# ChampiB/CBO_with_OOP

Hardware: AMD Instinct MI355X
Metric: candidate-intervention acquisitions/sec (16k grid, d=3) (higher is better)
Workload: dtype f64

## Files before the change

### cbo_with_oop_amd/GaussianProcessFactory.py

```python
from __future__ import annotations

import ctypes
import os
import warnings
from enum import IntEnum

import numpy as np

from . import _lib


class GaussianProcessType(IntEnum):
    GRAPH_GP = 0
    CAUSAL_GP = 1
    NON_CAUSAL_GP = 2


_LOGEXP_LIM = 36.0
_LOGEXP_LOG_LIM = float(np.log(np.finfo(np.float64).max))


def logexp_f(x):
    x = np.asarray(x, dtype=np.float64)
    return np.where(x > _LOGEXP_LIM, x, np.log1p(np.exp(np.clip(x, -_LOGEXP_LOG_LIM, _LOGEXP_LIM))))
# ... 93 lines not shown

    def _fit(self):
        tries = ctypes.c_int(0)
        jitter = ctypes.c_double(0.0)
        _lib.check(self._lib.cbo_gp_fit(self._handle, ctypes.byref(tries), ctypes.byref(jitter)))
        self._note_jitter(tries.value, jitter.value)

    def fit_level(self, level):
        status = ctypes.c_int(0)
        jitter = ctypes.c_double(0.0)
        _lib.check(self._lib.cbo_gp_fit_level(self._handle, int(level), ctypes.byref(status), ctypes.byref(jitter)))
        if status.value == 1:
            self._note_jitter(int(level), jitter.value)
        return status.value, jitter.value

    def adopted_factor(self, level):
        tries = ctypes.c_int(0)
        jitter = ctypes.c_double(0.0)
        _lib.check(self._lib.cbo_gp_jitter(self._handle, ctypes.byref(tries), ctypes.byref(jitter)))
        self._note_jitter(tries.value, jitter.value)

    def take_factor_slices(self, source, level, n_owners):
        _lib.check(self._lib.cbo_gp_take_factor_slices(self._handle, source._handle, int(level), int(n_owners)))
        self.adopted_factor(level)
        self.stale = False

    stale = False

    @property
    def small(self):
# ... 721 lines not shown
```

### cbo_with_oop_amd/_lib.py

```python
from __future__ import annotations

import atexit
import ctypes
import os
import threading
import weakref

import numpy as np

_HERE = os.path.dirname(os.path.abspath(__file__))
LIB_PATH = os.environ.get("CBO_HIP_LIB", os.path.join(_HERE, "libcbo_hip.so"))

c_double_p = ctypes.POINTER(ctypes.c_double)
c_int64_p = ctypes.POINTER(ctypes.c_int64)
c_int_p = ctypes.POINTER(ctypes.c_int)
c_void_pp = ctypes.POINTER(ctypes.c_void_p)

ABI_VERSION = 5
MAX_DIM = 8
MAX_APPEND = 64
MAX_HYPER_SAMPLES = 256
MAX_BATCH = 64
SMALL_BATCH_MAX_CANDS = 1024
CBO_OK = 0
# ... 222 lines not shown
    "cbo_acq_refine_sets_prior": (ctypes.c_int, [ctypes.c_int, c_void_pp, ctypes.POINTER(CboRefineSet), c_void_pp, ctypes.c_int,
                                                 c_double_p, ctypes.c_int, ctypes.c_double, ctypes.c_int, c_double_p, c_double_p,
                                                 c_double_p, c_int_p, c_int_p]),
    "cbo_do_prior_create": (ctypes.c_int, [ctypes.c_void_p, ctypes.c_int64, c_double_p, ctypes.c_int, c_int_p, c_void_pp]),
    "cbo_do_prior_destroy": (None, [ctypes.c_void_p]),
    "cbo_do_prior_eval": (ctypes.c_int, [ctypes.c_void_p, ctypes.c_int64, c_double_p, c_double_p, c_double_p]),
    "cbo_gp_hmc_sets": (ctypes.c_int, [ctypes.c_int, c_void_pp, ctypes.POINTER(CboHmcChain), c_int_p]),
    "cbo_gp_mle_sets": (ctypes.c_int, [ctypes.c_int, c_void_pp, ctypes.POINTER(CboMleRun), c_int_p]),
    "cbo_gp_mle_sets_rows": (ctypes.c_int, [ctypes.c_int, c_void_pp, ctypes.POINTER(CboMleRun), ctypes.c_int, c_int_p]),
    "cbo_gp_set_priors": (ctypes.c_int, [ctypes.c_void_p, ctypes.c_int, ctypes.POINTER(CboHyperPrior)]),
    "cbo_gp_get_priors": (ctypes.c_int, [ctypes.c_void_p, ctypes.c_int, ctypes.POINTER(CboHyperPrior)]),
    "cbo_gp_log_prior_batch": (ctypes.c_int, [ctypes.c_int, c_void_pp, ctypes.POINTER(c_double_p), c_double_p, c_double_p,
                                              c_int_p]),
    "cbo_gp_mes_gumbel_sets": (ctypes.c_int, [ctypes.c_int, c_void_pp, c_void_pp, c_double_p, c_double_p, c_double_p]),
    "cbo_gp_fit_level": (ctypes.c_int, [ctypes.c_void_p, ctypes.c_int, c_int_p, c_double_p]),
    "cbo_comm_gather_i64": (ctypes.c_int, [ctypes.c_void_p, ctypes.c_int64, c_int64_p]),
    "cbo_comm_share_factor": (ctypes.c_int, [ctypes.c_void_p, ctypes.c_void_p, ctypes.c_int, c_int_p, ctypes.c_int,
                                              c_int_p, ctypes.c_int]),
    "cbo_gp_take_factor_slices": (ctypes.c_int, [ctypes.c_void_p, ctypes.c_void_p, ctypes.c_int, ctypes.c_int]),
    "cbo_schedule_report": (ctypes.c_int, [ctypes.c_void_p, ctypes.c_char_p, ctypes.c_int64]),
    "cbo_trial_step": (ctypes.c_int, [ctypes.c_int, c_void_pp, c_void_pp, ctypes.c_int, ctypes.c_int64, c_double_p, c_double_p,
                                      c_double_p, c_double_p, c_double_p, ctypes.c_int, ctypes.c_double, c_double_p, c_double_p,
                                      c_int64_p, c_int_p]),
    "cbo_trial_step_kind": (ctypes.c_int, [ctypes.c_int, c_void_pp, c_void_pp, ctypes.c_int, ctypes.c_int64, c_double_p,
                                           c_double_p, c_double_p, c_double_p, ctypes.c_int, c_double_p, ctypes.c_int,
                                           ctypes.c_double, c_double_p, c_double_p, c_int64_p, c_int_p]),
    "cbo_acq_sweep_host": (ctypes.c_int, [ctypes.c_void_p, ctypes.c_int64, c_double_p, c_double_p, c_double_p,
                                          ctypes.c_double, ctypes.c_int, ctypes.c_double, ctypes.c_double,
                                          c_double_p, c_double_p, c_int64_p]),
    "cbo_argmax_sets": (ctypes.c_int, [c_double_p, ctypes.c_int, c_int_p]),
# ... 167 lines not shown
```

### cbo_with_oop_amd/csrc/cbo_api.hip

```cpp
#include <algorithm>
#include <atomic>
#include <cmath>
#include <cstdio>
#include <cstdlib>
#include <chrono>
#include <cstring>
#include <mutex>
#include <string>
#include <map>
#include <utility>
#include <vector>

#include "cbo_internal.h"
#include "hyper_prior.h"
#include "lml_outputs.h"
#include "schedule_tuner.h"

using namespace cbo;

static thread_local std::string g_err;
static std::atomic<uint64_t> g_fit_stamp{0};

static int fail(int code, const std::string &msg)
{
    g_err = msg;
    return code;
}
namespace cbo {
int set_error(int code, const std::string &msg) { return fail(code, msg); }
}

// ... 45 lines not shown
struct cbo_ctx {
    int device = 0;
    hipStream_t stream = nullptr;
    hipStream_t side_stream = nullptr;
    hipStream_t sweep_stream = nullptr;
    hipStream_t bulk_stream = nullptr;
    std::vector<hipEvent_t> chol_events;
    std::vector<hipEvent_t> pipe_events;
    hipEvent_t ev_join = nullptr, ev_join2 = nullptr, ev_fork = nullptr;
    hipEvent_t region_a = nullptr, region_b = nullptr;
    double pipe_tail_frac = -1.0;
    int pipe_group = 0;
    int pipe_lead = -1;
    CholOptions chol;
    int vec_solve_form = 2;
    int n_cu = 256;
    int n_cu_pipe = 256;
    ScheduleTable schedule;
    int64_t fused_fallbacks = 0;
    bool sweep_cache = true;
    bool small_sets = true;
    int sweep_mode = -1;
    int overlap_mode = -1;
    bool profiling = false;
    std::vector<EventPair> pending;
    EventPair pipe_cur{};
    std::vector<hipEvent_t> pool;
    cbo_timers timers{};
    GrowBuf<double> V;
    GrowBuf<double> W;
// ... 69 lines not shown
    double *y = nullptr, *ls_dev = nullptr;
    std::vector<double> ls;
    std::vector<double> h_pv;
    KernelHyper h{};
    double noise_var = 0.0;
    double *A = nullptr;
    double *invDt = nullptr;
    double *alpha = nullptr;
    double *z = nullptr;
    int *info = nullptr;
    bool fitted = false;
    uint64_t fit_stamp = 0;
    bool alpha_ready = false;
    int tries = 0;
    double jitter = 0.0;
    uint64_t parent_stamp = 0;
    double append_d = 0.0, append_zn = 0.0;
    double *lvec = nullptr;
    cbo_cands *probe = nullptr;
    int k_last = 1;
    int blk_side = 0;
    int64_t blk_rows = 0;
    double *blk_mem = nullptr;
    double *blk_B[2] = {nullptr, nullptr};
    double *blk_L22[2] = {nullptr, nullptr};
    double *blk_zb[2] = {nullptr, nullptr};
    double *blk_y[2] = {nullptr, nullptr};
    double *blk_Kbb[2] = {nullptr, nullptr};
    double *blk_part = nullptr;
    int *blk_status = nullptr;
// ... 207 lines not shown
    if (tf) c->pipe_tail_frac = std::atof(tf);
    const char *pg = std::getenv("CBO_HIP_PIPE_GROUP");
    if (pg) c->pipe_group = std::min(std::max(std::atoi(pg), 0), 4);
    const char *pl = std::getenv("CBO_HIP_PIPE_LEAD");
    if (pl) c->pipe_lead = std::atoi(pl);
    const char *pf = std::getenv("CBO_HIP_PANEL_FORM");
    if (pf && (std::atoi(pf) == 2 || std::atoi(pf) == 5)) c->chol.panel_form = std::atoi(pf);
    const char *sl = std::getenv("CBO_HIP_FUSED_SPIN_LIMIT");
    if (sl) c->chol.spin_limit = std::atoi(sl);
    const char *bg = std::getenv("CBO_HIP_BULK_GROUP");
    if (bg) c->chol.bulk_group = std::atoi(bg);
    const char *g4 = std::getenv("CBO_HIP_BULK_GROUP4_ROWS");
    if (g4) c->chol.group4_rows = std::atoi(g4);
    const char *vf = std::getenv("CBO_HIP_VEC_SOLVE_FORM");
    if (vf) c->vec_solve_form = std::atoi(vf);
    {
        static std::once_flag once;
        std::call_once(once, [] { std::atexit(shutdown_all_at_exit); });
        std::lock_guard<std::mutex> lock(g_live_mutex);
        g_live.push_back(c);
    }
    *out = c;
    return CBO_OK;
}

namespace cbo {
hipStream_t ctx_stream(cbo_ctx *c) { return c->stream; }
int ctx_device(cbo_ctx *c) { return c->device; }
}

// ... 242 lines not shown
{
    if (!g) return fail(CBO_ERR_INVALID, "gp is NULL");
    if (!g->fitted) return fail(CBO_ERR_NOT_FITTED, "gp is not fitted");
    if (tries_out) *tries_out = g->tries;
    if (jitter_out) *jitter_out = g->jitter;
    return CBO_OK;
}

static CholOptions chol_options(const cbo_ctx *c, bool separate)
{
    CholOptions o = c->chol;
    if (separate) o.panel_form = 2;
    return o;
}

static void enqueue_factor(cbo_gp *g, double jitter, bool separate)
{
    cbo_ctx *c = g->ctx;
    {
        PhaseScope ps(c, PH_KXX);
        launch_kxx(c->stream, g->X, g->h, g->noise_var + kGpyDiagJitter, jitter, g->A, g->lda, g->n_pad);
        launch_rhs(c->stream, g->y, g->X.pm, g->n, g->A, g->lda, g->n_pad, g->info, cholesky_info_ints(g->n_pad));
    }
    {
        PhaseScope ps(c, PH_CHOL);
        launch_cholesky(c->stream, c->side_stream, c->chol_events, g->A, g->lda, g->n_pad, g->invDt, g->info,
                        chol_options(c, separate), nullptr, true);
    }
}

static bool jitter_step(double base, int *tries, double *jitter)
{
    *jitter = *tries == 0 ? base : *jitter * 10.0;
    ++*tries;
    return *tries <= 5 && std::isfinite(*jitter);
}

static int next_jitter(cbo_gp *g, int *tries, double *jitter)
{
    double base = 0.0;
    if (*tries == 0) {
        long double sum = 0.0L;
        bool nonpos = false;
        for (int64_t i = 0; i < g->n; ++i) {
            const double dv = g->h.variance + (g->h_pv.empty() ? 0.0 : g->h_pv[i]) + (g->noise_var + kGpyDiagJitter);
            if (!(dv > 0.0)) nonpos = true;
            sum += (long double)dv;
        }
        if (nonpos) return fail(CBO_ERR_NONPOS_DIAG, "not pd: non-positive diagonal elements");
        base = (double)(sum / (long double)g->n) * 1e-6;
    }
// ... 9 lines not shown
        HIP_TRY(hipGetLastError());
        HIP_TRY(hipMemcpyAsync(c->h_info, info, sizeof(int), hipMemcpyDeviceToHost, c->stream));
        HIP_TRY(hipStreamSynchronize(c->stream));
        if (*c->h_info == kCholFusedTimeout) {
            if (separate)
                return fail(CBO_ERR_HIP, "a fused diagonal + panel launch gave up waiting, and so did the separate-launch repeat");
            separate = true;
            ++c->fused_fallbacks;
            continue;
        }
        *pd = *c->h_info == 0;
        return CBO_OK;
    }
}

static void mark_fitted(cbo_gp *g, int tries, double jitter)
{
    g->fitted = true;
    g->fit_stamp = ++g_fit_stamp;
    g->parent_stamp = 0;
    g->alpha_ready = false;
    g->tries = tries;
    g->jitter = jitter;
    if (g->ctx->profiling) g->ctx->timers.n_fit += 1;
}

static int adopt_factor(cbo_gp *g, int tries, double jitter)
{
    cbo_ctx *c = g->ctx;
    HIP_TRY(hipMemcpy2DAsync(g->z, sizeof(double), g->A + g->n_pad, sizeof(double) * g->lda, sizeof(double),
                             (size_t)g->n_pad, hipMemcpyDeviceToDevice, c->stream));
    HIP_TRY(hipGetLastError());
    mark_fitted(g, tries, jitter);
    return CBO_OK;
}

extern "C" int cbo_gp_fit(cbo_gp *g, int *tries_out, double *jitter_out)
{
    if (!g) return fail(CBO_ERR_INVALID, "gp is NULL");
    if (g->n <= 0 || g->n_pad <= 0) return fail(CBO_ERR_INVALID, "gp holds no data (a previous upload failed)");
    cbo_ctx *c = g->ctx;
    HIP_TRY(hipSetDevice(c->device));
    g->fitted = false;
    double jitter = 0.0;
    int tries = 0;
    for (;;) {
        bool pd = false;
        int rc = attempt_factor(c, g->info, [&](bool separate) { enqueue_factor(g, jitter, separate); }, &pd);
        if (rc != CBO_OK) return rc;
        if (pd) break;
        rc = next_jitter(g, &tries, &jitter);
        if (rc != CBO_OK) return rc;
    }
    const int rc = adopt_factor(g, tries, jitter);
    if (rc != CBO_OK) return rc;
    if (tries_out) *tries_out = tries;
    if (jitter_out) *jitter_out = jitter;
    return CBO_OK;
}

static int ladder_jitter(cbo_gp *g, int level, double *jitter)
{
    *jitter = 0.0;
    int tries = 0;
    while (tries < level) {
// ... 4 lines not shown
}

extern "C" int cbo_gp_fit_level(cbo_gp *g, int level, int *status, double *jitter_out)
{
    if (!g || !status) return fail(CBO_ERR_INVALID, "NULL argument");
    if (g->n <= 0 || g->n_pad <= 0) return fail(CBO_ERR_INVALID, "gp holds no data (a previous upload failed)");
    if (level < 0) return fail(CBO_ERR_INVALID, "level must be >= 0");
    cbo_ctx *c = g->ctx;
    HIP_TRY(hipSetDevice(c->device));
    g->fitted = false;
    double jitter = 0.0;
    int rc = ladder_jitter(g, level, &jitter);
    if (rc == CBO_ERR_NONPOS_DIAG) { *status = -1; return CBO_OK; }
    if (rc != CBO_OK) return rc;
    bool pd = false;
    rc = attempt_factor(c, g->info, [&](bool separate) { enqueue_factor(g, jitter, separate); }, &pd);
    if (rc != CBO_OK) return rc;
    *status = pd ? 1 : 0;
    if (jitter_out) *jitter_out = jitter;
    return pd ? adopt_factor(g, level, jitter) : CBO_OK;
}

namespace cbo {
int gp_factor_view(cbo_gp *g, double **A, int64_t *lda, int64_t *n_pad, double **invDt, cbo_ctx **ctx)
{
    if (!g) return fail(CBO_ERR_INVALID, "gp is NULL");
    if (g->n <= 0 || g->n_pad <= 0) return fail(CBO_ERR_INVALID, "gp holds no data");
    *A = g->A; *lda = g->lda; *n_pad = g->n_pad; *invDt = g->invDt; *ctx = g->ctx;
    return CBO_OK;
}
bool gp_is_fitted_at(const cbo_gp *g, int level) { return g && g->fitted && g->tries == level; }
int gp_adopt_received_factor(cbo_gp *g, int level)
{
    HIP_TRY(hipSetDevice(g->ctx->device));
    double jitter = 0.0;
// ... 1208 lines not shown
        mubuf = k->mu;
        k->fit_stamp = 0;
    }
    const bool speculate = qbuf == k->q;
    SweepPipe pipe = make_pipe(g, Vws, ldv, k->m_pad, qbuf, mubuf);
    pipe.group = choice.group;
    int pairs = choice.pairs;
    pipe.lead = 0;
    if (pipe.group >= 2 && pairs >= 1 && pairs * 256 < (int)g->n_pad)
        pipe.lead = forced ? (c->pipe_lead > 0 ? c->pipe_lead : 0) : (c->pipe_lead >= 0 ? c->pipe_lead : pairs % pipe.group);
    pipe.tail_begin = pairs * 256;
    if (pipe.tail_begin > (int)g->n_pad) pipe.tail_begin = (int)g->n_pad;
    double jitter = 0.0;
    int tries = 0;
    bool separate = false;
    for (;;) {
        HIP_TRY(hipEventRecord(c->ev_fork, c->stream));
        HIP_TRY(hipStreamWaitEvent(c->sweep_stream, c->ev_fork, 0));
        {
            PhaseScope ps(c, PH_KXX);
            launch_kxx(c->stream, g->X, g->h, g->noise_var + kGpyDiagJitter, jitter, g->A, g->lda, g->n_pad);
            launch_rhs(c->stream, g->y, g->X.pm, g->n, g->A, g->lda, g->n_pad, g->info, cholesky_info_ints(g->n_pad));
        }
        {
            PhaseScope ps(c, PH_KSTAR, c->sweep_stream);
            launch_kstar(c->sweep_stream, g->X, k->P, 0, k->m_pad, g->h, Vws, ldv, g->n_pad);
        }
        launch_zero_pair(c->sweep_stream, qbuf, mubuf, k->m_pad);
        {
            PhaseScope ps(c, PH_CHOL);
            launch_cholesky(c->stream, c->side_stream, c->chol_events, g->A, g->lda, g->n_pad, g->invDt, g->info,
                            chol_options(c, separate), &pipe, true);
        }
        HIP_TRY(hipEventRecord(c->ev_join, c->sweep_stream));
        HIP_TRY(hipStreamWaitEvent(c->stream, c->ev_join, 0));
        HIP_TRY(hipEventRecord(c->ev_join2, c->bulk_stream));
        HIP_TRY(hipStreamWaitEvent(c->stream, c->ev_join2, 0));
        HIP_TRY(hipGetLastError());
        if (speculate) {
            rc = enqueue_finish(g, k, y_best, task, ei_jitter, cost, acq_out, mean_out, var_out, qbuf, mubuf, true, false);
            if (rc != CBO_OK) return rc;
        } else {
            HIP_TRY(hipMemcpyAsync(c->h_info, g->info, sizeof(int), hipMemcpyDeviceToHost, c->stream));
        }
        HIP_TRY(hipStreamSynchronize(c->stream));
        if (*c->h_info == 0) break;
        if (*c->h_info == kCholFusedTimeout) {
            if (separate)
                return fail(CBO_ERR_HIP, "a fused diagonal + panel launch gave up waiting, and so did the separate-launch repeat");
            separate = true;
            ++c->fused_fallbacks;
            continue;
        }
        rc = next_jitter(g, &tries, &jitter);
        if (rc != CBO_OK) return rc;
    }
    mark_fitted(g, tries, jitter);
    if (tries_out) *tries_out = tries;
    if (jitter_out) *jitter_out = jitter;
    if (Vws != c->V) { k->v_stamp = g->fit_stamp; k->v_rows = g->n; }
    if (qbuf == k->q) k->fit_stamp = g->fit_stamp;
    if (speculate) {
        if (acq_out || mean_out || var_out) {
            rc = copy_posterior_out(c, k, acq_out, mean_out, var_out);
            if (rc != CBO_OK) return rc;
            HIP_TRY(hipStreamSynchronize(c->stream));
        }
        complete_finish(c, best_val, best_idx);
// ... 2849 lines not shown
```

### cbo_with_oop_amd/csrc/cbo_internal.h

```cpp
#pragma once

#include <hip/hip_runtime.h>
#include <cstddef>
#include <cstdint>
#include <string>
#include <vector>

#include "cbo_hip.h"

namespace cbo {

typedef double d4 __attribute__((ext_vector_type(4)));
typedef double d2 __attribute__((ext_vector_type(2)));

#if defined(__HIP_DEVICE_COMPILE__) || defined(__HIPCC__)
typedef __attribute__((address_space(3))) void *lds_ptr_t;
__device__ __forceinline__ void glds16(const double *gsrc, unsigned lds_dst)
{
    unsigned keep;
    asm volatile("s_mov_b32 %0, m0\n\ts_mov_b32 m0, %2\n\ts_nop 0\n\tglobal_load_lds_dwordx4 %1, off\n\ts_mov_b32 m0, %0"
                 : "=&s"(keep)
                 : "v"(gsrc), "s"(lds_dst)
                 : "memory");
}
// ... 112 lines not shown
    std::vector<hipEvent_t> *events;
    void (*mark)(void *user, hipStream_t st, int begin, double flops);
    void *user;
};
constexpr int kCholFlagSlots = 1024;
constexpr int kCholFusedTimeout = -2147483647 - 1;
constexpr int kFusedSpinLimit = 1 << 22;
struct CholOptions {
    int panel_form = 4;
    int spin_limit = kFusedSpinLimit;
    int bulk_group = 4;
    int group4_rows = 10240;
};
void launch_cholesky(hipStream_t s, hipStream_t side, std::vector<hipEvent_t> &events, double *A, int64_t lda,
                     int64_t n_pad, double *invDt, int *info_dev, const CholOptions &opt, const SweepPipe *pipe = nullptr,
                     bool info_zeroed = false);
inline int cholesky_info_ints(int64_t n_pad)
{
    const int np = (int)(n_pad / 128);
    return 2 * np <= kCholFlagSlots ? 1 + 2 * np : 1;
}
void sweep_pipe_pair(const SweepPipe &pipe, hipStream_t chain, const double *A, int64_t lda, const double *invDt,
                     int64_t n_pad, int p, int r0, int klen);
void sweep_pipe_tail(const SweepPipe &pipe, hipStream_t chain, const double *A, int64_t lda, const double *invDt,
                     int64_t n_pad, int pairs_done);
void launch_backsolve(hipStream_t s, const double *A, int64_t lda, int64_t n_pad, const double *invDt, double *alpha);
void launch_forward_vec(hipStream_t s, const double *A, int64_t lda, int64_t n_pad, const double *invDt, double *w,
                        double *out);
void launch_gather_column(hipStream_t s, const double *V, int64_t ldv, int64_t n_pad, double *dst);
bool launch_backsolve_chain(hipStream_t s, const double *A, int64_t lda, int64_t n_pad, const double *invDt,
                            const double *src, int64_t src_stride, double *work, double *out, int *info, int spin_limit,
// ... 362 lines not shown
```

### cbo_with_oop_amd/csrc/kernels_chol.hip

```cpp
#include <hip/hip_ext.h>
#include <climits>
#include <atomic>
#include <cstring>
#include <vector>

#include "cbo_mid_lml_device.h"

namespace cbo {

__global__ __launch_bounds__(256) void potrf_diag128_v2_kernel(double *A, int64_t lda, int r0, int rcol,
                                                               double *__restrict__ invDt, int *info,
                                                               double *__restrict__ zvec)
{
    extern __shared__ __align__(16) unsigned char smem_raw[];
    Diag2Shared &sh = *reinterpret_cast<Diag2Shared *>(smem_raw);
    if (__builtin_nontemporal_load(info) != 0) return;
    const int tid = threadIdx.x;
    const int lane = tid & 63;
    const int wave = __builtin_amdgcn_readfirstlane(tid >> 6);
    {
        const unsigned s0 = lds_byte_address(&sh.S[0][0]);
        const double *g = A + (int64_t)(r0 + wave * 32) * lda + r0 + lane * 2;
#pragma unroll 8
        for (int p = 0; p < 32; ++p) {
// ... 157 lines not shown
            for (int kk = 0; kk < 4; ++kk)
#pragma unroll
                for (int t = s + 1; t < 8; ++t) ub[kk][t] = coherent_load(Ub + (int64_t)(16 * s + 4 * kk) * lda + 16 * t);
        }
        const d4 nx = -x;
#pragma unroll
        for (int kk = 0; kk < 4; ++kk)
#pragma unroll
            for (int t = s + 1; t < 8; ++t) acc[t] = MFMA_F64(ub[kk][t], nx[kk], acc[t]);
    }
}

void launch_panel_fused(hipStream_t s, double *A, int64_t lda, int r0, int rcol, double *invDt, int *info, double *zvec,
                        int n_cols, int *flag, int spin_limit, hipEvent_t done = nullptr, bool split = false)
{
    if (!split) {
        hipExtLaunchKernelGGL(potrf_panel_fused_kernel, dim3(1u + (unsigned)(n_cols / kStrip)), dim3(256), sizeof(Diag2Shared),
                              s, nullptr, done, 0, A, lda, r0, rcol, invDt, info, zvec, r0 + 128, flag, spin_limit, 1);
        return;
    }
    hipLaunchKernelGGL(potrf_panel_fused_kernel, dim3(1u), dim3(256), sizeof(Diag2Shared), s, A, lda, r0, rcol, invDt, info,
                       zvec, r0 + 128, flag, spin_limit, 1);
    hipExtLaunchKernelGGL(potrf_panel_fused_kernel, dim3((unsigned)(n_cols / kStrip)), dim3(256), 0, s, nullptr, done, 0, A,
                          lda, r0, rcol, invDt, info, zvec, r0 + 128, flag, spin_limit, 0);
}

void launch_panel_trsm(hipStream_t s, double *A, int64_t lda, int r0, int col0, int n_cols, const double *invDt,
                       const int *skip_if, hipEvent_t done = nullptr)
{
    if (n_cols <= 0) { if (done) hipEventRecord(done, s); return; }
    hipExtLaunchKernelGGL(panel_trsm_kernel, dim3((unsigned)(n_cols / kStrip)), dim3(256), sizeof(PanelShared), s, nullptr,
// ... 375 lines not shown
    const double rows = (double)((int)n_pad - t0);
    if (pipe.mark) pipe.mark(pipe.user, chain, 1, rows * rows * (double)pipe.m_pad);
    launch_trsm_strips(chain, A + (int64_t)t0 * lda + t0, lda, invDt + (int64_t)(t0 / 16) * 256,
                       pipe.V + (int64_t)t0 * pipe.ldv, pipe.ldv, (int64_t)n_pad - t0, pipe.m_pad, pipe.zvec + t0, pipe.q,
                       pipe.mu, true, false);
    if (pipe.mark) pipe.mark(pipe.user, chain, 0, 0.0);
}

__global__ void zero_ints_kernel(int *p, int n)
{
    for (int i = threadIdx.x; i < n; i += blockDim.x) p[i] = 0;
}

void launch_cholesky(hipStream_t s, hipStream_t side, std::vector<hipEvent_t> &events, double *A, int64_t lda,
                     int64_t n_pad, double *invDt, int *info_dev, const CholOptions &opt, const SweepPipe *pipe,
                     bool info_zeroed)
{
    hipFuncSetAttribute(reinterpret_cast<const void *>(potrf_diag128_v2_kernel), hipFuncAttributeMaxDynamicSharedMemorySize,
                        (int)sizeof(Diag2Shared));
    hipFuncSetAttribute(reinterpret_cast<const void *>(panel_trsm_kernel), hipFuncAttributeMaxDynamicSharedMemorySize,
                        (int)sizeof(PanelShared));
    hipFuncSetAttribute(reinterpret_cast<const void *>(potrf_panel_fused_kernel), hipFuncAttributeMaxDynamicSharedMemorySize,
                        (int)sizeof(Diag2Shared));
    constexpr int syrk_gemm_rows = 6144;
    auto launch_diag = [&](int rr) {
        hipLaunchKernelGGL(potrf_diag128_v2_kernel, dim3(1), dim3(256), sizeof(Diag2Shared), s, A, lda, rr, (int)n_pad,
                           invDt, info_dev, pipe ? pipe->zvec : nullptr);
    };
    const int np = (int)(n_pad / 128);
    const bool fused = opt.panel_form != 2 && 2 * np <= kCholFlagSlots;
    const bool split = opt.panel_form == 5;
    if (!info_zeroed) hipLaunchKernelGGL(zero_ints_kernel, dim3(1), dim3(256), 0, s, info_dev, fused ? 1 + 2 * np : 1);
    int *flags = info_dev + 1;
    const int rcol = (int)n_pad;
    event_slot(events, (size_t)(2 * np + 1));
    hipEventRecord(events[2 * np], s);
    hipStreamWaitEvent(side, events[2 * np], 0);
    double *zvec = pipe ? pipe->zvec : nullptr;
    const bool lean_panel = !pipe;
    int pair = 0;
    auto sweep_rows = [&](int r0, int klen) {
        if (pipe && r0 < pipe->tail_begin) sweep_pipe_pair(*pipe, s, A, lda, invDt, n_pad, pair++, r0, klen);
    };
    int pending = -1;
    int group_left = 0;
    int group_pairs = 0, group_g0 = 0, group_first_k = 0;
    int pending_big_a = -1;
    for (int k = 0; k < np; k += 2) {
        const int r0 = 128 * k;
        const int n2 = (int)n_pad - r0 - 128;
        const int n3_pair = (int)n_pad - r0 - 256;
        if (group_left == 0 && opt.bulk_group >= 2 && (fused || lean_panel)) {
            int G = 0;
            if (opt.bulk_group >= 4 && n3_pair - 1024 >= opt.group4_rows && n3_pair - 1024 >= syrk_gemm_rows &&
                n3_pair - 1024 >= 1024)
                G = 4;
            else if (n3_pair - 512 >= syrk_gemm_rows && n3_pair - 512 >= 512) G = 2;
            if (G != 0) { group_pairs = G; group_left = G; group_g0 = r0; group_first_k = k; }
        }
        const bool grouped = group_left > 0;
        const bool first_of_group = grouped && group_left == group_pairs;
        const bool last_of_group = grouped && group_left == 1;
        const bool split_now = split || grouped;
        auto factor_panel = [&](int r, int cols, hipEvent_t done) {
            if (fused && cols > 0) {
                launch_panel_fused(s, A, lda, r, rcol, invDt, info_dev, zvec, cols, flags + 2 * (r / 128), opt.spin_limit,
                                   done, split_now);
                return;
            }
            launch_diag(r);
            if (cols <= 0) return;
            if (lean_panel) launch_panel_trsm(s, A, lda, r, r + 128, cols, invDt, info_dev, done);
            else
                launch_trsm_strips(s, A + (int64_t)r * lda + r, lda, invDt + (int64_t)(r / 16) * 256,
                                   A + (int64_t)r * lda + r + 128, lda, 128, cols, nullptr, nullptr, nullptr, false, true);
        };
        factor_panel(r0, n2, nullptr);
        if (n2 <= 0) { sweep_rows(r0, 128); break; }
        launch_syrk_rows(s, A, lda, r0, 128, n2, rcol, info_dev);
        const int r1 = r0 + 128;
        const int n3 = (int)n_pad - r1 - 128;
        const bool bulk = n3 > 256;
        const bool gemm_form = bulk && n3 - 256 >= syrk_gemm_rows;
        const bool carried = bulk && (fused || lean_panel);
        const hipEvent_t ev_panel = (carried && gemm_form && (!grouped || last_of_group)) ? events[2 * k] : nullptr;
        const hipEvent_t ev_rows = (carried && !gemm_form) ? events[2 * k] : nullptr;
        factor_panel(r1, n3, ev_panel);
        sweep_rows(r0, 256);
        if (n3 <= 0) break;
        if (grouped) {
            const int S = 256 * group_pairs, g0 = group_g0, n = (int)n_pad;
            const int next_end = (g0 + 2 * S < n) ? g0 + 2 * S : n;
            if (last_of_group) {
                hipStreamWaitEvent(side, events[2 * k], 0);
                const int a_end = (g0 + 3 * S < n) ? g0 + 3 * S : n;
                launch_gemm_update(side, A, lda, A, lda, A, lda, g0, S, next_end, a_end, n_pad + kRhsCols, true, info_dev);
                hipEventRecord(events[2 * group_first_k + 1], side);
                pending_big_a = 2 * group_first_k + 1;
                if (a_end < n)
                    launch_gemm_update(side, A, lda, A, lda, A, lda, g0, S, a_end, n, n_pad + kRhsCols, true, info_dev);
                hipEventRecord(events[2 * k + 1], side);
                pending = 2 * k + 1;
            }
            launch_syrk_rows(s, A, lda, r0, 256, n3, rcol, info_dev, 256, nullptr);
            if (first_of_group && pending_big_a >= 0) hipStreamWaitEvent(s, events[pending_big_a], 0);
            launch_gemm_update(s, A, lda, A, lda, A, lda, r0, 256, r0 + 512, next_end, n_pad + kRhsCols, true, info_dev);
            --group_left;
            continue;
        }
        const int prev = pending;
        auto launch_bulk = [&] {
            if (!carried) hipEventRecord(events[2 * k], s);
            hipStreamWaitEvent(side, events[2 * k], 0);
            if (gemm_form)
                launch_gemm_update(side, A, lda, A, lda, A, lda, r0, 256, r0 + 256 + 256, (int)n_pad, n_pad + kRhsCols, true,
                                   info_dev);
            else
                launch_syrk(side, A, lda, r0, 256, n3, rcol, 4, n3 / 64, info_dev);
            hipEventRecord(events[2 * k + 1], side);
            pending = 2 * k + 1;
        };
        if (gemm_form) launch_bulk();
        if (prev >= 0) hipStreamWaitEvent(s, events[prev], 0);
        launch_syrk_rows(s, A, lda, r0, 256, n3, rcol, info_dev, 256, ev_rows);
        if (bulk && !gemm_form) launch_bulk();
    }
    hipEventRecord(events[2 * np + 1], side);
    hipStreamWaitEvent(s, events[2 * np + 1], 0);
    if (pipe && pipe->tail_begin < (int)n_pad) sweep_pipe_tail(*pipe, s, A, lda, invDt, n_pad, pair);
}

__global__ __launch_bounds__(256) void backsolve_step_kernel(const double *__restrict__ A, int64_t lda,
                                                             const double *__restrict__ invDt, int blk, double *zt,
                                                             double *__restrict__ alpha)
{
    __shared__ double zs[128];
    __shared__ double al[128];
    const int tid = threadIdx.x;
    const int lane = tid & 63, wave = tid >> 6;
    const int b0 = blk * 128;
    if (tid < 128) zs[tid] = zt[b0 + tid];
    __syncthreads();
    for (int s = 7; s >= 0; --s) {
        const int o = 16 * s;
// ... 317 lines not shown
```

### include/cbo_hip.h

```cpp
#ifndef CBO_HIP_H
#define CBO_HIP_H

#include <stdint.h>

#ifdef __cplusplus
extern "C" {
#endif

#define CBO_HIP_ABI_VERSION 5
#define CBO_MAX_DIM 8

typedef enum cbo_status {
    CBO_OK = 0,
    CBO_ERR_INVALID = -1,
    CBO_ERR_HIP = -2,
    CBO_ERR_NOT_PD = -3,
    CBO_ERR_NONPOS_DIAG = -4,
    CBO_ERR_NOT_FITTED = -5,
    CBO_ERR_UNSUPPORTED = -6,
    CBO_ERR_NO_DEVICE = -7,
    CBO_ERR_COMM = -8
} cbo_status;

enum { CBO_DTYPE_F64 = 0, CBO_DTYPE_F32 = 1 };
// ... 148 lines not shown

int cbo_acq_sweep_batch_logei(cbo_gp *gp, cbo_cands *cands, double y_best, int task, double jitter, double cost,
                              int batch_size, int update_incumbent, double *best_vals, int64_t *best_idxs, double *acq_out,
                              double *mean_out, double *var_out);

int cbo_gp_fit_sweep(cbo_gp *gp, cbo_cands *cands, double y_best, int task, double ei_jitter, double cost,
                     double *acq_out, double *mean_out, double *var_out, double *best_val,
                     int64_t *best_idx, int *tries_out, double *jitter_out);

int cbo_acq_sweep_sets(int n_sets, cbo_gp *const *gps, cbo_cands *const *cands, const double *y_best, int task,
                       double ei_jitter, const double *costs, double *best_vals, int64_t *best_idxs);

int cbo_schedule_report(cbo_ctx *ctx, char *buf, int64_t cap);

int cbo_gp_fit_level(cbo_gp *gp, int level, int *status, double *jitter_out);

int cbo_trial_step(int n_sets, cbo_gp *const *gps, cbo_cands *const *cands, int refit_set, int64_t n,
                   const double *X, const double *y, const double *prior_mean_X, const double *prior_var_X,
                   const double *y_best, int task, double ei_jitter, const double *costs, double *best_vals,
                   int64_t *best_idxs, int *chosen_out);

int cbo_acq_sweep_sets_kind(int n_sets, cbo_gp *const *gps, cbo_cands *const *cands, int kind, const double *y_best,
                            int task, double param, const double *costs, double *best_vals, int64_t *best_idxs);
int cbo_trial_step_kind(int n_sets, cbo_gp *const *gps, cbo_cands *const *cands, int refit_set, int64_t n,
                        const double *X, const double *y, const double *prior_mean_X, const double *prior_var_X,
                        int kind, const double *y_best, int task, double param, const double *costs, double *best_vals,
                        int64_t *best_idxs, int *chosen_out);

int cbo_acq_sweep_sets_logei(int n_sets, cbo_gp *const *gps, cbo_cands *const *cands, const double *y_best, int task,
                             double jitter, const double *costs, double *best_vals, int64_t *best_idxs);
// ... 169 lines not shown
```

Baseline: 3.070 million.

## Probe jitter ladder levels with partial leading-block Cholesky before full refactor

Remembers, per jitter level, the pivot at which the previous Cholesky failed. On the next fit it first factors only the leading rows up to that pivot, rounded to 256, and moves to the next jitter level if that smaller factor still fails. This avoids paying for a full-size factorization that is likely to fail. The partial factor reuses the Cholesky launcher with a row limit, which adds bookkeeping and an extra probe launch when the hint is stale. It also adds probe and report API entry points.

Measured after the change: 3.081 million, median of 6. About the same (+0.3%).

```diff
diff --git a/cbo_with_oop_amd/GaussianProcessFactory.py b/cbo_with_oop_amd/GaussianProcessFactory.py
--- a/cbo_with_oop_amd/GaussianProcessFactory.py
+++ b/cbo_with_oop_amd/GaussianProcessFactory.py
@@ -131,6 +131,26 @@
             self._note_jitter(int(level), jitter.value)
         return status.value, jitter.value
 
+    def probe_level(self, level, rows, want_factor=False):
+        status = ctypes.c_int(0)
+        pivot = ctypes.c_int(0)
+        out = np.empty((int(rows), int(rows))) if want_factor else None
+        _lib.check(self._lib.cbo_gp_probe_level(self._handle, int(level), int(rows), ctypes.byref(status), ctypes.byref(pivot),
+                                                _lib.dptr(out)))
+        self.stale = True
+        return status.value, pivot.value, (out if want_factor and status.value == 1 else None)
+
+    def fit_report(self):
+        cap = 16
+        n = ctypes.c_int(0)
+        level = (ctypes.c_int * cap)()
+        rows = (ctypes.c_int64 * cap)()
+        status = (ctypes.c_int * cap)()
+        hints = (ctypes.c_int * 6)()
+        _lib.check(self._lib.cbo_gp_fit_report(self._handle, cap, ctypes.byref(n), level, rows, status, hints))
+        k = min(n.value, cap)
+        return {"attempts": [(level[i], rows[i], status[i]) for i in range(k)], "hints": list(hints)}
+
     def adopted_factor(self, level):
         tries = ctypes.c_int(0)
         jitter = ctypes.c_double(0.0)
diff --git a/cbo_with_oop_amd/_lib.py b/cbo_with_oop_amd/_lib.py
--- a/cbo_with_oop_amd/_lib.py
+++ b/cbo_with_oop_amd/_lib.py
@@ -260,6 +260,8 @@
                                               c_int_p]),
     "cbo_gp_mes_gumbel_sets": (ctypes.c_int, [ctypes.c_int, c_void_pp, c_void_pp, c_double_p, c_double_p, c_double_p]),
     "cbo_gp_fit_level": (ctypes.c_int, [ctypes.c_void_p, ctypes.c_int, c_int_p, c_double_p]),
+    "cbo_gp_probe_level": (ctypes.c_int, [ctypes.c_void_p, ctypes.c_int, ctypes.c_int64, c_int_p, c_int_p, c_double_p]),
+    "cbo_gp_fit_report": (ctypes.c_int, [ctypes.c_void_p, ctypes.c_int, c_int_p, c_int_p, c_int64_p, c_int_p, c_int_p]),
     "cbo_comm_gather_i64": (ctypes.c_int, [ctypes.c_void_p, ctypes.c_int64, c_int64_p]),
     "cbo_comm_share_factor": (ctypes.c_int, [ctypes.c_void_p, ctypes.c_void_p, ctypes.c_int, c_int_p, ctypes.c_int,
                                               c_int_p, ctypes.c_int]),
diff --git a/cbo_with_oop_amd/csrc/cbo_api.hip b/cbo_with_oop_amd/csrc/cbo_api.hip
--- a/cbo_with_oop_amd/csrc/cbo_api.hip
+++ b/cbo_with_oop_amd/csrc/cbo_api.hip
@@ -15,6 +15,7 @@
 #include "hyper_prior.h"
 #include "lml_outputs.h"
 #include "schedule_tuner.h"
+#include "fit_ladder.h"
 
 using namespace cbo;
 
@@ -90,6 +91,7 @@
     int pipe_lead = -1;
     CholOptions chol;
     int vec_solve_form = 2;
+    int fit_probe = FIT_PROBE_DEFAULT;
     int n_cu = 256;
     int n_cu_pipe = 256;
     ScheduleTable schedule;
@@ -189,6 +191,8 @@
     bool alpha_ready = false;
     int tries = 0;
     double jitter = 0.0;
+    FitHints hints;
+    std::vector<FitAttempt> attempts;
     uint64_t parent_stamp = 0;
     double append_d = 0.0, append_zn = 0.0;
     double *lvec = nullptr;
@@ -426,6 +430,8 @@
     if (g4) c->chol.group4_rows = std::atoi(g4);
     const char *vf = std::getenv("CBO_HIP_VEC_SOLVE_FORM");
     if (vf) c->vec_solve_form = std::atoi(vf);
+    const char *fp = std::getenv("CBO_HIP_FIT_PROBE");
+    if (fp && std::atoi(fp) >= FIT_PROBE_NEVER && std::atoi(fp) <= FIT_PROBE_ANY_SIZE) c->fit_probe = std::atoi(fp);
     {
         static std::once_flag once;
         std::call_once(once, [] { std::atexit(shutdown_all_at_exit); });
@@ -698,27 +704,21 @@
     return o;
 }
 
-static void enqueue_factor(cbo_gp *g, double jitter, bool separate)
+static void enqueue_factor(cbo_gp *g, double jitter, bool separate, int64_t rows)
 {
     cbo_ctx *c = g->ctx;
     {
         PhaseScope ps(c, PH_KXX);
-        launch_kxx(c->stream, g->X, g->h, g->noise_var + kGpyDiagJitter, jitter, g->A, g->lda, g->n_pad);
-        launch_rhs(c->stream, g->y, g->X.pm, g->n, g->A, g->lda, g->n_pad, g->info, cholesky_info_ints(g->n_pad));
+        launch_kxx(c->stream, g->X, g->h, g->noise_var + kGpyDiagJitter, jitter, g->A, g->lda, rows);
+        launch_rhs(c->stream, g->y, g->X.pm, std::min(g->n, rows), g->A, g->lda, rows, g->info, cholesky_info_ints(g->n_pad));
     }
     {
         PhaseScope ps(c, PH_CHOL);
         launch_cholesky(c->stream, c->side_stream, c->chol_events, g->A, g->lda, g->n_pad, g->invDt, g->info,
-                        chol_options(c, separate), nullptr, true);
-    }
-}
-
-static bool jitter_step(double base, int *tries, double *jitter)
-{
-    *jitter = *tries == 0 ? base : *jitter * 10.0;
-    ++*tries;
-    return *tries <= 5 && std::isfinite(*jitter);
-}
+                        chol_options(c, separate), nullptr, true, rows);
+    }
+}
+
 
 static int next_jitter(cbo_gp *g, int *tries, double *jitter)
 {
@@ -758,6 +758,21 @@
     }
 }
 
+static int run_probes(cbo_gp *g, FitWalk &walk, int *tries, double *jitter)
+{
+    cbo_ctx *c = g->ctx;
+    for (int64_t rows; (rows = walk.next_rows()) < g->n_pad;) {
+        bool pd = false;
+        int rc = attempt_factor(c, g->info, [&](bool separate) { enqueue_factor(g, *jitter, separate, rows); }, &pd);
+        if (rc != CBO_OK) return rc;
+        if (walk.report(rows, *c->h_info) == FitWalk::NEXT_LEVEL) {
+            rc = next_jitter(g, tries, jitter);
+            if (rc != CBO_OK) return rc;
+        }
+    }
+    return CBO_OK;
+}
+
 static void mark_fitted(cbo_gp *g, int tries, double jitter)
 {
     g->fitted = true;
@@ -788,11 +803,14 @@
     g->fitted = false;
     double jitter = 0.0;
     int tries = 0;
+    FitWalk walk(g->hints, g->n_pad, c->fit_probe, &g->attempts);
     for (;;) {
+        int rc = run_probes(g, walk, &tries, &jitter);
+        if (rc != CBO_OK) return rc;
         bool pd = false;
-        int rc = attempt_factor(c, g->info, [&](bool separate) { enqueue_factor(g, jitter, separate); }, &pd);
+        rc = attempt_factor(c, g->info, [&](bool separate) { enqueue_factor(g, jitter, separate, g->n_pad); }, &pd);
         if (rc != CBO_OK) return rc;
-        if (pd) break;
+        if (walk.report(g->n_pad, *c->h_info) == FitWalk::DONE) break;
         rc = next_jitter(g, &tries, &jitter);
         if (rc != CBO_OK) return rc;
     }
@@ -827,11 +845,54 @@
     if (rc == CBO_ERR_NONPOS_DIAG) { *status = -1; return CBO_OK; }
     if (rc != CBO_OK) return rc;
     bool pd = false;
-    rc = attempt_factor(c, g->info, [&](bool separate) { enqueue_factor(g, jitter, separate); }, &pd);
+    rc = attempt_factor(c, g->info, [&](bool separate) { enqueue_factor(g, jitter, separate, g->n_pad); }, &pd);
     if (rc != CBO_OK) return rc;
     *status = pd ? 1 : 0;
     if (jitter_out) *jitter_out = jitter;
     return pd ? adopt_factor(g, level, jitter) : CBO_OK;
+}
+
+extern "C" int cbo_gp_probe_level(cbo_gp *g, int level, int64_t rows, int *status, int *pivot, double *factor_out)
+{
+    if (!g || !status) return fail(CBO_ERR_INVALID, "NULL argument");
+    if (g->n <= 0 || g->n_pad <= 0) return fail(CBO_ERR_INVALID, "gp holds no data (a previous upload failed)");
+    if (level < 0) return fail(CBO_ERR_INVALID, "level must be >= 0");
+    if (rows <= 0 || rows % kFitProbeRowStep != 0 || rows > g->n_pad)
+        return fail(CBO_ERR_INVALID, "rows must be a positive multiple of 256, at most the model's padded row count");
+    cbo_ctx *c = g->ctx;
+    HIP_TRY(hipSetDevice(c->device));
+    g->fitted = false;
+    if (pivot) *pivot = 0;
+    double jitter = 0.0;
+    int rc = ladder_jitter(g, level, &jitter);
+    if (rc == CBO_ERR_NONPOS_DIAG) { *status = -1; return CBO_OK; }
+    if (rc != CBO_OK) return rc;
+    bool pd = false;
+    rc = attempt_factor(c, g->info, [&](bool separate) { enqueue_factor(g, jitter, separate, rows); }, &pd);
+    if (rc != CBO_OK) return rc;
+    *status = pd ? 1 : 0;
+    if (pivot && !pd) *pivot = *c->h_info;
+    if (pd && factor_out) {
+        HIP_TRY(hipMemcpy2DAsync(factor_out, sizeof(double) * (size_t)rows, g->A, sizeof(double) * (size_t)g->lda,
+                                 sizeof(double) * (size_t)rows, (size_t)rows, hipMemcpyDeviceToHost, c->stream));
+        HIP_TRY(hipStreamSynchronize(c->stream));
+        for (int64_t i = 1; i < rows; ++i)
+            for (int64_t j = 0; j < i; ++j) factor_out[i * rows + j] = 0.0;
+    }
+    return CBO_OK;
+}
+
+extern "C" int cbo_gp_fit_report(cbo_gp *g, int cap, int *n_attempts, int *level, int64_t *rows, int *status, int *hints)
+{
+    if (!g) return fail(CBO_ERR_INVALID, "gp is NULL");
+    if (n_attempts) *n_attempts = (int)g->attempts.size();
+    for (int i = 0; i < cap && i < (int)g->attempts.size(); ++i) {
+        if (level) level[i] = g->attempts[i].level;
+        if (rows) rows[i] = g->attempts[i].rows;
+        if (status) status[i] = g->attempts[i].status;
+    }
+    for (int l = 0; hints && l < kLadderLevels; ++l) hints[l] = g->hints.pivot[l];
+    return CBO_OK;
 }
 
 namespace cbo {
@@ -2070,7 +2131,10 @@
     double jitter = 0.0;
     int tries = 0;
     bool separate = false;
+    FitWalk walk(g->hints, g->n_pad, c->fit_probe, &g->attempts);
     for (;;) {
+        rc = run_probes(g, walk, &tries, &jitter);
+        if (rc != CBO_OK) return rc;
         HIP_TRY(hipEventRecord(c->ev_fork, c->stream));
         HIP_TRY(hipStreamWaitEvent(c->sweep_stream, c->ev_fork, 0));
         {
@@ -2100,7 +2164,6 @@
             HIP_TRY(hipMemcpyAsync(c->h_info, g->info, sizeof(int), hipMemcpyDeviceToHost, c->stream));
         }
         HIP_TRY(hipStreamSynchronize(c->stream));
-        if (*c->h_info == 0) break;
         if (*c->h_info == kCholFusedTimeout) {
             if (separate)
                 return fail(CBO_ERR_HIP, "a fused diagonal + panel launch gave up waiting, and so did the separate-launch repeat");
@@ -2108,6 +2171,7 @@
             ++c->fused_fallbacks;
             continue;
         }
+        if (walk.report(g->n_pad, *c->h_info) == FitWalk::DONE) break;
         rc = next_jitter(g, &tries, &jitter);
         if (rc != CBO_OK) return rc;
     }
diff --git a/cbo_with_oop_amd/csrc/cbo_internal.h b/cbo_with_oop_amd/csrc/cbo_internal.h
--- a/cbo_with_oop_amd/csrc/cbo_internal.h
+++ b/cbo_with_oop_amd/csrc/cbo_internal.h
@@ -150,7 +150,7 @@
 };
 void launch_cholesky(hipStream_t s, hipStream_t side, std::vector<hipEvent_t> &events, double *A, int64_t lda,
                      int64_t n_pad, double *invDt, int *info_dev, const CholOptions &opt, const SweepPipe *pipe = nullptr,
-                     bool info_zeroed = false);
+                     bool info_zeroed = false, int64_t rows = 0);
 inline int cholesky_info_ints(int64_t n_pad)
 {
     const int np = (int)(n_pad / 128);
diff --git a/cbo_with_oop_amd/csrc/fit_ladder.h b/cbo_with_oop_amd/csrc/fit_ladder.h
--- /dev/null
+++ b/cbo_with_oop_amd/csrc/fit_ladder.h
@@ -0,0 +1,80 @@
+#pragma once
+#include <cmath>
+#include <cstdint>
+#include <vector>
+
+
+constexpr int kLadderLevels = 6;
+
+constexpr int64_t kFitProbeMaxRowsNum = 7, kFitProbeMaxRowsDen = 8;
+constexpr int64_t kFitProbeMinRows = 2048;
+constexpr int64_t kFitProbeRowStep = 256;
+
+enum FitProbeMode { FIT_PROBE_NEVER = 0, FIT_PROBE_DEFAULT = 1, FIT_PROBE_ANY_SIZE = 2 };
+
+inline bool jitter_step(double base, int *tries, double *jitter)
+{
+    *jitter = *tries == 0 ? base : *jitter * 10.0;
+    ++*tries;
+    return *tries <= 5 && std::isfinite(*jitter);
+}
+
+struct FitHints {
+    int pivot[kLadderLevels] = {0, 0, 0, 0, 0, 0};
+};
+
+struct FitAttempt {
+    int level;
+    int64_t rows;
+    int status;
+};
+
+inline int64_t fit_probe_rows(int pivot, int64_t n_pad, int mode)
+{
+    if (pivot <= 0 || mode == FIT_PROBE_NEVER) return 0;
+    if (mode != FIT_PROBE_ANY_SIZE && n_pad < kFitProbeMinRows) return 0;
+    const int64_t rows = ((int64_t)pivot + kFitProbeRowStep - 1) / kFitProbeRowStep * kFitProbeRowStep;
+    if (rows * kFitProbeMaxRowsDen > n_pad * kFitProbeMaxRowsNum) return 0;
+    return rows;
+}
+
+struct FitWalk {
+    enum Result { DONE, SAME_LEVEL, NEXT_LEVEL };
+    FitHints &hints;
+    const int64_t n_pad;
+    const int mode;
+    std::vector<FitAttempt> *log;
+    int lvl = 0;
+    bool probed[kLadderLevels] = {false, false, false, false, false, false};
+
+    FitWalk(FitHints &h, int64_t n_pad_, int mode_, std::vector<FitAttempt> *log_ = nullptr)
+        : hints(h), n_pad(n_pad_), mode(mode_), log(log_)
+    {
+        if (log) log->clear();
+    }
+    int level() const { return lvl; }
+    int64_t next_rows() const
+    {
+        if (lvl >= kLadderLevels || probed[lvl]) return n_pad;
+        const int64_t rows = fit_probe_rows(hints.pivot[lvl], n_pad, mode);
+        return rows > 0 ? rows : n_pad;
+    }
+    Result report(int64_t rows, int status)
+    {
+        if (log) log->push_back(FitAttempt{lvl, rows, status});
+        const bool probe = rows < n_pad;
+        if (lvl >= kLadderLevels) return status == 0 && !probe ? DONE : NEXT_LEVEL;
+        if (probe) probed[lvl] = true;
+        if (status != 0) {
+            hints.pivot[lvl] = status > 0 ? status : 0;
+            ++lvl;
+            return NEXT_LEVEL;
+        }
+        if (probe) {
+            hints.pivot[lvl] = 0;
+            return SAME_LEVEL;
+        }
+        for (int l = lvl; l < kLadderLevels; ++l) hints.pivot[l] = 0;
+        return DONE;
+    }
+};
diff --git a/cbo_with_oop_amd/csrc/kernels_chol.hip b/cbo_with_oop_amd/csrc/kernels_chol.hip
--- a/cbo_with_oop_amd/csrc/kernels_chol.hip
+++ b/cbo_with_oop_amd/csrc/kernels_chol.hip
@@ -195,7 +195,7 @@
 void launch_panel_fused(hipStream_t s, double *A, int64_t lda, int r0, int rcol, double *invDt, int *info, double *zvec,
                         int n_cols, int *flag, int spin_limit, hipEvent_t done = nullptr, bool split = false)
 {
-    if (!split) {
+    if (!split || n_cols <= 0) {
         hipExtLaunchKernelGGL(potrf_panel_fused_kernel, dim3(1u + (unsigned)(n_cols / kStrip)), dim3(256), sizeof(Diag2Shared),
                               s, nullptr, done, 0, A, lda, r0, rcol, invDt, info, zvec, r0 + 128, flag, spin_limit, 1);
         return;
@@ -601,8 +601,10 @@
 
 void launch_cholesky(hipStream_t s, hipStream_t side, std::vector<hipEvent_t> &events, double *A, int64_t lda,
                      int64_t n_pad, double *invDt, int *info_dev, const CholOptions &opt, const SweepPipe *pipe,
-                     bool info_zeroed)
-{
+                     bool info_zeroed, int64_t rows)
+{
+    const int nf = (int)n_pad;
+    const int nr = (rows > 0 && rows < n_pad && !pipe) ? (int)rows : nf;
     hipFuncSetAttribute(reinterpret_cast<const void *>(potrf_diag128_v2_kernel), hipFuncAttributeMaxDynamicSharedMemorySize,
                         (int)sizeof(Diag2Shared));
     hipFuncSetAttribute(reinterpret_cast<const void *>(panel_trsm_kernel), hipFuncAttributeMaxDynamicSharedMemorySize,
@@ -611,15 +613,16 @@
                         (int)sizeof(Diag2Shared));
     constexpr int syrk_gemm_rows = 6144;
     auto launch_diag = [&](int rr) {
-        hipLaunchKernelGGL(potrf_diag128_v2_kernel, dim3(1), dim3(256), sizeof(Diag2Shared), s, A, lda, rr, (int)n_pad,
+        hipLaunchKernelGGL(potrf_diag128_v2_kernel, dim3(1), dim3(256), sizeof(Diag2Shared), s, A, lda, rr, nr,
                            invDt, info_dev, pipe ? pipe->zvec : nullptr);
     };
-    const int np = (int)(n_pad / 128);
-    const bool fused = opt.panel_form != 2 && 2 * np <= kCholFlagSlots;
+    const int np_full = nf / 128;
+    const int np = nr / 128;
+    const bool fused = opt.panel_form != 2 && 2 * np_full <= kCholFlagSlots;
     const bool split = opt.panel_form == 5;
     if (!info_zeroed) hipLaunchKernelGGL(zero_ints_kernel, dim3(1), dim3(256), 0, s, info_dev, fused ? 1 + 2 * np : 1);
     int *flags = info_dev + 1;
-    const int rcol = (int)n_pad;
+    const int rcol = nr;
     event_slot(events, (size_t)(2 * np + 1));
     hipEventRecord(events[2 * np], s);
     hipStreamWaitEvent(side, events[2 * np], 0);
@@ -635,8 +638,8 @@
     int pending_big_a = -1;
     for (int k = 0; k < np; k += 2) {
         const int r0 = 128 * k;
-        const int n2 = (int)n_pad - r0 - 128;
-        const int n3_pair = (int)n_pad - r0 - 256;
+        const int n2 = nr - r0 - 128;
+        const int n3_pair = nf - r0 - 256;
         if (group_left == 0 && opt.bulk_group >= 2 && (fused || lean_panel)) {
             int G = 0;
             if (opt.bulk_group >= 4 && n3_pair - 1024 >= opt.group4_rows && n3_pair - 1024 >= syrk_gemm_rows &&
@@ -650,7 +653,7 @@
         const bool last_of_group = grouped && group_left == 1;
         const bool split_now = split || grouped;
         auto factor_panel = [&](int r, int cols, hipEvent_t done) {
-            if (fused && cols > 0) {
+            if (fused && (cols > 0 || r + 128 < nf)) {
                 launch_panel_fused(s, A, lda, r, rcol, invDt, info_dev, zvec, cols, flags + 2 * (r / 128), opt.spin_limit,
                                    done, split_now);
                 return;
@@ -666,9 +669,10 @@
         if (n2 <= 0) { sweep_rows(r0, 128); break; }
         launch_syrk_rows(s, A, lda, r0, 128, n2, rcol, info_dev);
         const int r1 = r0 + 128;
-        const int n3 = (int)n_pad - r1 - 128;
-        const bool bulk = n3 > 256;
-        const bool gemm_form = bulk && n3 - 256 >= syrk_gemm_rows;
+        const int n3 = nr - r1 - 128;
+        const int n3_full = nf - r1 - 128;
+        const bool bulk = n3_full > 256;
+        const bool gemm_form = bulk && n3_full - 256 >= syrk_gemm_rows;
         const bool carried = bulk && (fused || lean_panel);
         const hipEvent_t ev_panel = (carried && gemm_form && (!grouped || last_of_group)) ? events[2 * k] : nullptr;
         const hipEvent_t ev_rows = (carried && !gemm_form) ? events[2 * k] : nullptr;
@@ -676,22 +680,22 @@
         sweep_rows(r0, 256);
         if (n3 <= 0) break;
         if (grouped) {
-            const int S = 256 * group_pairs, g0 = group_g0, n = (int)n_pad;
+            const int S = 256 * group_pairs, g0 = group_g0, n = nr;
             const int next_end = (g0 + 2 * S < n) ? g0 + 2 * S : n;
             if (last_of_group) {
                 hipStreamWaitEvent(side, events[2 * k], 0);
                 const int a_end = (g0 + 3 * S < n) ? g0 + 3 * S : n;
-                launch_gemm_update(side, A, lda, A, lda, A, lda, g0, S, next_end, a_end, n_pad + kRhsCols, true, info_dev);
+                launch_gemm_update(side, A, lda, A, lda, A, lda, g0, S, next_end, a_end, nr + kRhsCols, true, info_dev);
                 hipEventRecord(events[2 * group_first_k + 1], side);
                 pending_big_a = 2 * group_first_k + 1;
                 if (a_end < n)
-                    launch_gemm_update(side, A, lda, A, lda, A, lda, g0, S, a_end, n, n_pad + kRhsCols, true, info_dev);
+                    launch_gemm_update(side, A, lda, A, lda, A, lda, g0, S, a_end, n, nr + kRhsCols, true, info_dev);
                 hipEventRecord(events[2 * k + 1], side);
                 pending = 2 * k + 1;
             }
             launch_syrk_rows(s, A, lda, r0, 256, n3, rcol, info_dev, 256, nullptr);
             if (first_of_group && pending_big_a >= 0) hipStreamWaitEvent(s, events[pending_big_a], 0);
-            launch_gemm_update(s, A, lda, A, lda, A, lda, r0, 256, r0 + 512, next_end, n_pad + kRhsCols, true, info_dev);
+            launch_gemm_update(s, A, lda, A, lda, A, lda, r0, 256, r0 + 512, next_end, nr + kRhsCols, true, info_dev);
             --group_left;
             continue;
         }
@@ -700,8 +704,7 @@
             if (!carried) hipEventRecord(events[2 * k], s);
             hipStreamWaitEvent(side, events[2 * k], 0);
             if (gemm_form)
-                launch_gemm_update(side, A, lda, A, lda, A, lda, r0, 256, r0 + 256 + 256, (int)n_pad, n_pad + kRhsCols, true,
-                                   info_dev);
+                launch_gemm_update(side, A, lda, A, lda, A, lda, r0, 256, r0 + 256 + 256, nr, nr + kRhsCols, true, info_dev);
             else
                 launch_syrk(side, A, lda, r0, 256, n3, rcol, 4, n3 / 64, info_dev);
             hipEventRecord(events[2 * k + 1], side);
@@ -714,7 +717,7 @@
     }
     hipEventRecord(events[2 * np + 1], side);
     hipStreamWaitEvent(s, events[2 * np + 1], 0);
-    if (pipe && pipe->tail_begin < (int)n_pad) sweep_pipe_tail(*pipe, s, A, lda, invDt, n_pad, pair);
+    if (pipe && pipe->tail_begin < nf) sweep_pipe_tail(*pipe, s, A, lda, invDt, n_pad, pair);
 }
 
 __global__ __launch_bounds__(256) void backsolve_step_kernel(const double *__restrict__ A, int64_t lda,
diff --git a/include/cbo_hip.h b/include/cbo_hip.h
--- a/include/cbo_hip.h
+++ b/include/cbo_hip.h
@@ -186,6 +186,9 @@
 int cbo_schedule_report(cbo_ctx *ctx, char *buf, int64_t cap);
 
 int cbo_gp_fit_level(cbo_gp *gp, int level, int *status, double *jitter_out);
+
+int cbo_gp_probe_level(cbo_gp *gp, int level, int64_t rows, int *status, int *pivot, double *factor_out);
+int cbo_gp_fit_report(cbo_gp *gp, int cap, int *n_attempts, int *level, int64_t *rows, int *status, int *hints);
 
 int cbo_trial_step(int n_sets, cbo_gp *const *gps, cbo_cands *const *cands, int refit_set, int64_t n,
                    const double *X, const double *y, const double *prior_mean_X, const double *prior_var_X,
```
